# NethermindEth/starkpack-winterfell

Measured on AMD Instinct MI355X. Metric: trace-LDE + Merkle-commit field-ops/s (wall-clock ms in ms_per_step), 2^20x8 f64 trace blowup=8, higher is better.
Workload: dtype u64 (Goldilocks, Montgomery form) + u32 (BLAKE3)

## Files before the change

### starkpack-winterfell_amd/csrc/context.hip

```cpp
#include "wf_internal.hpp"

#include <atomic>

#include "field.hpp"

using namespace wf;

static thread_local char g_err[512] = "";

std::atomic<uint64_t> g_fail_epoch{0};
uint64_t fail_epoch() { return g_fail_epoch.load(std::memory_order_relaxed); }

int fail(int code, const char *fmt, ...) {
    g_fail_epoch.fetch_add(1, std::memory_order_relaxed);
    va_list ap;
    va_start(ap, fmt);
    vsnprintf(g_err, sizeof(g_err), fmt, ap);
    va_end(ap);
    return code;
}

const char *last_error_text() { return g_err; }

wf_tuning tuning_from_env() {
// ... 2 lines not shown
    if (!on || strcmp(on, "1") != 0) return t;
    if (const char *e = getenv("WF_EXP_MAX_DIGIT")) {
        const int v = atoi(e);
        if (v >= 4 && v <= 11) t.max_digit = (uint32_t)v;
    }
    t.no_specialized = getenv("WF_EXP_NO_SPECIALIZED") != nullptr;
    t.full_tiles = getenv("WF_EXP_FULL_TILES") != nullptr;
    t.no_fused_hash = getenv("WF_EXP_NO_FUSED_HASH") != nullptr;
    t.no_chunked = getenv("WF_EXP_NO_CHUNKED") != nullptr;
    t.persistent_always = getenv("WF_EXP_PERSISTENT_ALWAYS") != nullptr;
    t.no_persistent = getenv("WF_EXP_NO_PERSISTENT") != nullptr;
    if (const char *e = getenv("WF_EXP_MERKLE_L2_MIN")) {
        const int v = atoi(e);
        if (v >= 10 && v <= 30) t.merkle_l2_min = (uint32_t)v;
    }
    t.no_pipeline = getenv("WF_EXP_NO_PIPELINE") != nullptr;
    t.no_tail_pack = getenv("WF_EXP_NO_TAIL_PACK") != nullptr;
    t.no_coset_inner = getenv("WF_EXP_NO_COSET_INNER") != nullptr;
    t.no_gtab = getenv("WF_EXP_NO_GTAB") != nullptr;
    t.no_staged_chunks = getenv("WF_EXP_NO_STAGED_CHUNKS") != nullptr;
    t.no_gtab1 = getenv("WF_EXP_NO_GTAB1") != nullptr;
    t.no_ftab = getenv("WF_EXP_NO_FTAB") != nullptr;
    t.no_gtab1_wide = getenv("WF_EXP_NO_GTAB1_WIDE") != nullptr;
    t.gtab1_f64 = getenv("WF_EXP_GTAB1_F64") != nullptr;
    if (const char *e = getenv("WF_EXP_WIDE_TI")) {
        const int v = atoi(e);
        if (v == 1 || v == 2 || v == 4 || v == 8) t.wide_ti = (uint32_t)v;
    }
    if (const char *e = getenv("WF_EXP_PIPELINE_MIN_BYTES")) {
        const long long v = atoll(e);
        if (v >= 0 && v <= (1ll << 40)) t.pipeline_min_bytes = (size_t)v;
    }
    if (const char *e = getenv("WF_EXP_FAIL_AFTER_SEGMENT")) {
        const int v = atoi(e);
        if (v >= 0 && v < 4096) t.fail_after_segment = v;
    }
    if (const char *e = getenv("WF_EXP_GRIND_WINDOW_LOG2")) {
        const int v = atoi(e);
        if (v >= 2 && v <= 30) t.grind_window_log2 = (uint32_t)v;
    }
    if (const char *e = getenv("WF_EXP_GRIND_WINDOW_CAP_LOG2")) {
        const int v = atoi(e);
        if (v >= 2 && v <= 30) t.grind_window_cap_log2 = (uint32_t)v;
    }
    return t;
}
// ... 395 lines not shown
```

### starkpack-winterfell_amd/csrc/path.hip

```cpp
#include "wf_internal.hpp"

#include "kernels.hpp"
#include "keccak_dev.hpp"
#include "keccak_kernels.hpp"
#include "merkle_plan.hpp"
#include "rescue_kernels.hpp"
#include "rescue_jive_kernels.hpp"
#include "griffin_dev.hpp"
#include "seg_kernels.hpp"
#include "col_kernels.hpp"
#include "fri_kernels.hpp"
#include "tables.hpp"

using namespace wf;

#if defined(WF_EXPERIMENTS) && defined(WF_EXP_STAMPS)
static unsigned long long *g_exp_stamps = nullptr;
static unsigned long long *exp_stamps_buffer() {
    if (!g_exp_stamps && hipMalloc(&g_exp_stamps, 4096 * 8 * 8) == hipSuccess) (void)hipMemset(g_exp_stamps, 0, 4096 * 8 * 8);
    return g_exp_stamps;
}
extern "C" int wf_exp_stamps_read(unsigned long long *out, int clear) {
    if (!g_exp_stamps) return -1;
    if (hipMemcpy(out, g_exp_stamps, 4096 * 8 * 8, hipMemcpyDeviceToHost) != hipSuccess) return -2;
// ... 181 lines not shown
    return true;
}

template <class F>
struct SegDesc {
    typedef typename F::T T;
    const T *in;
    T *work;
    T *out;
    uint32_t logN, n_seg, n_cosets;
    bool rows_out;
    void *leaves = nullptr;
    uint32_t hash_epr = 0;
    uint32_t digest_words = 8;
    bool *fused = nullptr;
    const TableSet *pre;
    const T *fin_tab = nullptr;
    bool pad_traces = false;
    bool pad_in_kernel = false;
    uint32_t base_cols, total_base_cols, coset0;
    uint64_t row_width, trace_lde_elems;
    uint32_t seg0 = 0, seg_cnt = 0;
    int phase = 0;
};

template <class F>
static int run_seg_transform(wf_ctx *ctx, hipStream_t st, const SegDesc<F> &d) {
    typedef typename F::T T;
    const bool inverse = !d.rows_out;
    TableSet *tw;
    int rc = root_tables<F>(ctx, d.logN, inverse, &tw);
    if (rc) return rc;
    const Plan plan = seg_plan<F>(d.logN, d.n_seg, ctx->tune.max_digit, ctx->tune.full_tiles);
    const uint64_t N = (uint64_t)1 << d.logN;

    SegArgs<F> a;
    memset(&a, 0, sizeof(a));
    a.logN = d.logN;
    a.n_seg = d.n_seg;
    a.n_cosets = d.n_cosets;
    a.tw = as_pow2l<F>(*tw);
    if (d.pre) {
        a.pre = as_pow2l<F>(*d.pre);
        a.pre_lo_stride = d.pre->lo_stride;
        a.pre_hi_stride = d.pre->hi_stride;
    }
// ... 29 lines not shown
        const uint64_t tickets_tp = (uint64_t)(d.n_cosets / 2) << (d.logN - logDl);
        const uint64_t launch_rows = (uint64_t)d.n_cosets << d.logN;
        tailpack = logDl >= (ctx->tune.persistent_always || F::BYTES == 16 ? 7u : 9u) && logDl <= 10 && tickets_tp % 8 == 0 &&
                   tickets_tp < (1ull << 31) &&
                   (ctx->tune.persistent_always || launch_rows >= (1ull << 20));
    }
    T *work_tail = tailpack ? d.work + (size_t)d.n_cosets * nf * N * S_ : nullptr;

    const uint32_t run_cnt = tailpack ? nf : (d.seg_cnt ? d.seg_cnt : d.n_seg);
    const size_t run_off = (size_t)d.seg0 * (N * SegCfg<F>::S);
    a.seg_stride = tailpack ? nf : d.n_seg;
    uint32_t done_bits = 0;
    for (int pi = 0; pi + 1 < plan.n_pass; pi++) {
        if (d.phase == 2) {
            done_bits += plan.dig[pi];
            continue;
        }
        const bool first = pi == 0;
        a.logD = plan.dig[pi];
        a.O = (uint64_t)1 << done_bits;
        a.I = N >> (done_bits + a.logD);
        rc = digit_table<F>(ctx, a.logD, inverse, &a.digit_tw);
        if (rc) return rc;
        if (d.rows_out) {
            a.src = first ? d.in : d.work;
            a.dst = d.work;
            a.src_shared = first ? 1 : 0;
            a.pre_on = first ? 1 : 0;
            a.scale_on = 0;
        } else {
            a.src = first ? d.in : d.work;
            a.dst = d.work;
            a.src_shared = 0;
            a.pre_on = 0;
            a.scale_on = first ? 1 : 0;
            a.scale = inv_n;
        }
        a.src += run_off;
        a.dst += run_off;
        a.n_seg = run_cnt;
        uint32_t threads;
        size_t lds;
        rc = seg_launch_dims<F>(a.logD, threads, lds, false);
        if (rc) return rc;
        const uint64_t grid = (uint64_t)n_groups * run_cnt * a.O * a.I;
        if (grid > 0x7FFFFFFFull) return fail(WF_ERR_ARG, "problem too large for one launch (%llu groups)", (unsigned long long)grid);
// ... 90 lines not shown
    }
    a.n_seg = d.n_seg;
    a.seg_stride = d.n_seg;
    a.coset_inner = 0;
    a.fout_tab = nullptr;
    if (d.phase == 1) return 0;
    {
        const int pi = plan.n_pass - 1;
        const bool single = plan.n_pass == 1;
        a.logD = plan.dig[pi];
        a.O = (uint64_t)1 << done_bits;
        a.I = 1;
        a.n_prev = plan.n_pass - 1;
        for (int i = 0; i < pi; i++) a.prev_log[i] = plan.dig[i];
        rc = digit_table<F>(ctx, a.logD, inverse, &a.digit_tw);
        if (rc) return rc;
        a.src = single ? d.in : d.work;
        a.dst = d.out;
        a.src_shared = (single && d.rows_out) ? 1 : 0;
        a.pre_on = (single && d.rows_out) ? 1 : 0;
        a.fin_tab = (single && d.rows_out && !packed) ? d.fin_tab : nullptr;
        a.scale_on = (single && !d.rows_out) ? 1 : 0;
        a.scale = inv_n;
        uint32_t threads;
        size_t lds;
        rc = seg_launch_dims<F>(a.logD, threads, lds, true);
        if (rc) return rc;
        const uint64_t grid = (uint64_t)n_groups * d.n_seg * a.O;
        if (grid > 0x7FFFFFFFull) return fail(WF_ERR_ARG, "problem too large for one launch (%llu groups)", (unsigned long long)grid);
        const bool fuse_on = d.rows_out && d.leaves && !ctx->tune.no_fused_hash;
        const bool may_fuse = fuse_on && !packed;
        const bool chunked = d.n_seg > 16 && !ctx->tune.no_chunked;
        const uint32_t n_chunks = chunked ? (d.n_seg + 15) / 16 : 1;
        const uint64_t tickets = (uint64_t)d.n_cosets * a.O * n_chunks;
        const uint64_t launch_rows = (uint64_t)d.n_cosets << d.logN;
        const bool one_seg = d.n_seg == 1 && d.total_base_cols == d.base_cols;
        const bool always = ctx->tune.persistent_always;
        const bool persistent = may_fuse && !single && (d.n_seg <= 16 || chunked) && threads * 2 == (1u << a.logD) &&
                                (always || !one_seg || a.logD >= 10) &&
                                (always || one_seg || chunked || d.total_base_cols != d.base_cols || launch_rows >= (1ull << 20)) &&
                                tickets % 8 == 0 && tickets < (1ull << 31) && launch_rows * n_chunks * 32 < (1ull << 40) &&
                                !ctx->tune.no_persistent;
        const bool fuse_packed = fuse_on && packed && (F::BYTES == 16 || a.lg_log >= 2 || d.total_base_cols != d.base_cols);
        const bool fuse = persistent || (may_fuse && d.n_seg == 1 && d.total_base_cols == d.base_cols) || fuse_packed;
        a.leaves = fuse ? (uint32_t *)d.leaves : nullptr;
        a.hash_epr = d.hash_epr;
// ... 66 lines not shown
#endif
            void *kargs[] = {&a};
            HIP_TRY(hipLaunchKernel(kern, dim3((uint32_t)std::min<uint64_t>(tickets, resident)), dim3(threads), kargs, lds_p, st));
            if (chunked) {
                HIP_TRY(hipGetLastError());
                launch_merge_chunks(st, ctx->hash_tmp.p, n_chunks, launch_rows, d.leaves, a.digest_words);
            }
        } else if (d.rows_out && packed)
            hipLaunchKernelGGL((k_seg_last<F, SEG_OUT_ROWS, true>), dim3((uint32_t)grid), dim3(threads), lds, st, a);
        else {
            const void *kern = d.rows_out ? (const void *)k_seg_last<F, SEG_OUT_ROWS> : (const void *)k_seg_last<F, SEG_OUT_SEG>;
            constexpr bool F8 = F::BYTES == 8;
            if (F8 && threads * 2 == (1u << a.logD) && !ctx->tune.no_specialized) {
                if (a.logD == 10)
                    kern = d.rows_out ? (const void *)k_seg_last<F, SEG_OUT_ROWS, false, F8 ? 10 : 0> : (const void *)k_seg_last<F, SEG_OUT_SEG, false, F8 ? 10 : 0>;
                else if (a.logD == 9)
                    kern = d.rows_out ? (const void *)k_seg_last<F, SEG_OUT_ROWS, false, F8 ? 9 : 0> : (const void *)k_seg_last<F, SEG_OUT_SEG, false, F8 ? 9 : 0>;
            }
            if (lds > 64 * 1024) HIP_TRY(hipFuncSetAttribute(kern, hipFuncAttributeMaxDynamicSharedMemorySize, 160 * 1024));
            void *kargs[] = {&a};
            HIP_TRY(hipLaunchKernel(kern, dim3((uint32_t)grid), dim3(threads), kargs, lds, st));
        }
        HIP_TRY(hipGetLastError());
    }
    return 0;
}

template <class F>
static int run_xpose(wf_ctx *ctx, hipStream_t st, bool to_seg, const void *src, void *dst, uint64_t R, uint32_t W,
                     uint32_t total_base_cols, uint32_t n_seg, uint32_t seg0 = 0, uint32_t seg_cnt = 0) {
    if (seg_cnt == 0) seg_cnt = n_seg - seg0;
    XposeArgs<F> x;
    x.seg0 = seg0;
    x.src = (const typename F::T *)src;
    x.dst = (typename F::T *)dst;
    x.R = R;
    x.W = W;
    x.total_base_cols = total_base_cols;
    constexpr uint32_t RPB = XPOSE_TILES * 256 / SegCfg<F>::S;
    const uint64_t grid = (uint64_t)seg_cnt * ((R + RPB - 1) / RPB);
    if (grid > 0x7FFFFFFFull) return fail(WF_ERR_ARG, "problem too large for one launch");
    prof_mark(ctx, st, to_seg ? "layout.cols_to_segments" : "layout.segments_to_cols");
    if (to_seg)
        hipLaunchKernelGGL(k_cols_to_seg<F>, dim3((uint32_t)grid), dim3(256), 0, st, x);
    else
        hipLaunchKernelGGL(k_seg_to_cols<F>, dim3((uint32_t)grid), dim3(256), 0, st, x);
// ... 194 lines not shown
    d.seg0 = seg0;
    d.seg_cnt = seg_cnt;
    rc = run_seg_transform<F>(ctx, st, d);
    if (rc) return rc;
    if (phase == 1) return 0;

    if (d_leaves) {
        if (!hashed) {
            prof_mark(ctx, st, "hash_rows");
            rc = run_hash_rows<F>(ctx, st, d_lde, Nrows * row_width, Nrows, (uint32_t)row_width, base_cols, p->n_traces, d_leaves, p->hasher, p->digest_bytes);
            if (rc) return rc;
        }
        if (d_nodes) {
            prof_mark(ctx, st, "merkle");
            rc = run_merkle(ctx, st, d_leaves, Nrows, d_nodes, p->hasher, p->digest_bytes);
            if (rc) return rc;
        }
    }
    prof_mark(ctx, st, "between_calls");
    return 0;
}

template <class F>
static int trace_commit_dev(wf_ctx *ctx, const wf_params *p, const void *d_trace, void *d_polys, void *d_lde,
                            void *d_leaves, void *d_nodes, hipStream_t st, hipEvent_t input_read = nullptr) {
    PathBufs<F> b;
    int rc = path_buffers<F>(ctx, p, b);
    if (rc) return rc;
    const uint64_t R = (uint64_t)1 << p->log2_trace_len;
    rc = run_xpose<F>(ctx, st, true, d_trace, b.segA, R, p->ext_degree, b.total_base_cols, b.n_seg);
    if (rc) return rc;
    if (input_read) HIP_TRY(hipEventRecord(input_read, st));
    SegDesc<F> d;
    memset(&d, 0, sizeof(d));
    d.in = b.segA;
    d.work = b.segA;
    d.out = b.segB;
    d.logN = p->log2_trace_len;
    d.n_seg = b.n_seg;
    d.n_cosets = 1;
    d.rows_out = false;
    rc = run_seg_transform<F>(ctx, st, d);
    if (rc) return rc;
    rc = run_xpose<F>(ctx, st, false, b.segB, d_polys, R, p->ext_degree, b.total_base_cols, b.n_seg);
    if (rc) return rc;
    return evaluate_and_commit<F>(ctx, st, p, b, d_lde, d_leaves, d_nodes);
}

template <class F>
static int trace_commit_pipelined_impl(wf_ctx *ctx, const wf_params *p, const void *const *cols_in, void *d_stage, void *d_polys,
                                       void *d_lde, void *d_leaves, void *d_nodes, hipStream_t st, void *const *polys_out) {
    typedef typename F::T T;
    constexpr uint32_t S = SegCfg<F>::S;
    PathBufs<F> b;
    int rc = path_buffers<F>(ctx, p, b);
    if (rc) return rc;
    const uint64_t R = (uint64_t)1 << p->log2_trace_len;
    const size_t colb = R * sizeof(T), TC = b.total_base_cols;
    if (!ctx->copy_stream) HIP_TRY(hipStreamCreateWithFlags(&ctx->copy_stream, hipStreamNonBlocking));
    while (ctx->seg_events.size() < (size_t)b.n_seg + 1) {
        hipEvent_t e;
        HIP_TRY(hipEventCreateWithFlags(&e, hipEventDisableTiming));
        ctx->seg_events.push_back(e);
    }
    HIP_TRY(hipEventRecord(ctx->seg_events[b.n_seg], st));
// ... 107 lines not shown

int wf_constraint_commit_dev(wf_ctx *ctx, const wf_params *p, const void *d_polys, void *d_lde, void *d_leaves,
                             void *d_nodes, void *stream) {
    if (!ctx) return fail(WF_ERR_ARG, "ctx is null");
    int rc = check_params(p, true);
    if (rc) return rc;
    if (!d_polys || !d_lde) return fail(WF_ERR_ARG, "null device buffer");
    HIP_TRY(hipSetDevice(ctx->device));
    hipStream_t st = stream ? (hipStream_t)stream : ctx->stream;
    WF_ENTER(ctx, st);
    if (p->field == WF_FIELD_F64) return constraint_commit_dev<F64>(ctx, p, d_polys, d_lde, d_leaves, d_nodes, st);
    return constraint_commit_dev<F128>(ctx, p, d_polys, d_lde, d_leaves, d_nodes, st);
}

}

template <class F>
static int trace_commit_shard_dev(wf_ctx *ctx, const wf_params *p, uint32_t coset0, uint32_t n_cosets,
                                  const void *d_trace, void *d_polys, void *d_lde, void *d_leaves, hipStream_t st) {
    PathBufs<F> b;
    int rc = path_buffers<F>(ctx, p, b, n_cosets);
    if (rc) return rc;
    const uint64_t R = (uint64_t)1 << p->log2_trace_len;
    rc = run_xpose<F>(ctx, st, true, d_trace, b.segA, R, p->ext_degree, b.total_base_cols, b.n_seg);
    if (rc) return rc;
    SegDesc<F> d;
    memset(&d, 0, sizeof(d));
    d.in = b.segA;
    d.work = b.segA;
    d.out = b.segB;
    d.logN = p->log2_trace_len;
    d.n_seg = b.n_seg;
    d.n_cosets = 1;
    d.rows_out = false;
    rc = run_seg_transform<F>(ctx, st, d);
    if (rc) return rc;
    if (d_polys) {
        rc = run_xpose<F>(ctx, st, false, b.segB, d_polys, R, p->ext_degree, b.total_base_cols, b.n_seg);
        if (rc) return rc;
    }
    return evaluate_and_commit<F>(ctx, st, p, b, d_lde, d_leaves, nullptr, coset0, n_cosets);
}

extern "C" {

int wf_trace_commit_shard_dev(wf_ctx *ctx, const wf_params *p, uint32_t coset_begin, uint32_t coset_count,
                              const void *d_trace, void *d_polys, void *d_lde_shard, void *d_leaves_shard,
                              void *stream) {
    if (!ctx) return fail(WF_ERR_ARG, "ctx is null");
    int rc = check_params(p, false);
    if (rc) return rc;
    if ((rc = check_blake3_only(p, "wf_trace_commit_shard_dev"))) return rc;
    if (!d_trace || !d_lde_shard || !d_leaves_shard) return fail(WF_ERR_ARG, "null device buffer");
    const uint32_t blowup = 1u << p->log2_blowup;
    if (coset_count == 0 || coset_begin >= blowup || coset_count > blowup - coset_begin)
        return fail(WF_ERR_ARG, "coset range [%u, %u) is not inside [0, %u)", coset_begin, coset_begin + coset_count, blowup);
    HIP_TRY(hipSetDevice(ctx->device));
    hipStream_t st = stream ? (hipStream_t)stream : ctx->stream;
// ... 425 lines not shown
```

### starkpack-winterfell_amd/csrc/seg_kernels.hpp

```cpp
#pragma once

#include <hip/hip_runtime.h>
#include <stdint.h>

#include "field.hpp"
#include "kernels.hpp"

#ifndef WF_EXPERIMENTS
#undef WF_EXP_SKIP_LOAD
#undef WF_EXP_SKIP_NTT
#undef WF_EXP_SKIP_STORE
#undef WF_EXP_LOCAL_STORE
#undef WF_EXP_STAMPS
#endif

namespace wf {

template <class F>
struct SegCfg {
    static constexpr uint32_t S = 64 / F::BYTES;
    static constexpr uint32_t HP = S / 2;
    static constexpr bool RADIX16 = F::BYTES == 8;
    static constexpr bool RADIX8 = F::BYTES == 16;
    static constexpr uint32_t LOAD_BATCH = F::BYTES == 8 ? 8 : 4;
};

template <class T>
struct alignas(16) Pair {
// ... 11 lines not shown
    if (z & 1) {
        *pz++ = F::zero();
        z++;
    }
    const Pair<typename F::T> zz{F::zero(), F::zero()};
    for (; z < row_width; z += 2, pz += 2) store_pair(pz, zz);
}

template <class F>
__device__ __forceinline__ Pair<typename F::T> pair_from(const uint4 &qa, const uint4 &qb);
template <>
__device__ __forceinline__ Pair<uint64_t> pair_from<F64>(const uint4 &qa, const uint4 &) {
    Pair<uint64_t> v;
    v.a = ((uint64_t)qa.y << 32) | qa.x;
    v.b = ((uint64_t)qa.w << 32) | qa.z;
    return v;
}
template <>
__device__ __forceinline__ Pair<U128> pair_from<F128>(const uint4 &qa, const uint4 &qb) {
    Pair<U128> v;
    v.a = U128{((uint64_t)qa.y << 32) | qa.x, ((uint64_t)qa.w << 32) | qa.z};
    v.b = U128{((uint64_t)qb.y << 32) | qb.x, ((uint64_t)qb.w << 32) | qb.z};
    return v;
}

enum : int { SEG_OUT_SEG = 0, SEG_OUT_ROWS = 1 };

template <int LOGD>
__device__ __forceinline__ uint32_t tile_threads() {
    return LOGD ? (1u << (LOGD ? LOGD - 1 : 0)) : blockDim.x;
}
#define WF_TILE_BOUNDS(LOGD, GENERIC) __launch_bounds__((LOGD) ? (1 << ((LOGD) ? (LOGD) - 1 : 0)) : (GENERIC), (LOGD) ? 4 : 1)

__device__ __forceinline__ uint64_t xcd_group_index(uint64_t b, uint64_t total) {
    if ((total & 63) != 0) return b;
    const uint64_t xcd = b & 7, seq = b >> 3;
    return (((seq >> 3) << 3) + xcd) * 8 + (seq & 7);
}

__device__ __forceinline__ uint64_t coset_inner_split(uint64_t bid, uint32_t lc, uint32_t &c) {
    const uint64_t hi = bid >> 6;
    c = (uint32_t)hi & ((1u << lc) - 1);
    return ((hi >> lc) << 6) | (bid & 63);
}

__device__ __forceinline__ uint32_t ilog2_pow2(uint64_t v) { return 63u - (uint32_t)__builtin_clzll(v); }
// ... 20 lines not shown
    uint32_t scale_on;
    T scale;
    uint32_t n_prev;
    uint32_t prev_log[3];
    uint32_t base_cols;
    uint32_t total_base_cols;
    uint32_t store_cols, total_store_cols;
    uint32_t pad_traces;
    uint32_t tail_pad;
    uint32_t seg_stride;
    uint32_t coset0;
    uint32_t rows_per_k;
    uint32_t cpr_log, lg_log;
    uint64_t row_width;
    uint64_t trace_lde_elems;
    uint32_t *leaves;
    uint32_t hash_epr;
    uint32_t digest_words;
    uint32_t *chunk_cvs;
    uint32_t n_chunks;
    uint32_t *tile_counters;
    const T *src_tail;
    uint32_t tail_cols;
#ifdef WF_EXP_STAMPS
    unsigned long long *stamps;
#endif
};

#if defined(WF_EXPERIMENTS) && defined(WF_EXP_R8_NO_SPLIT)
constexpr uint32_t R8_SPLIT = 0;
#else
constexpr uint32_t R8_SPLIT = 4;
#endif
__host__ __device__ constexpr uint32_t radix8_rounds(uint32_t logD) {
    return (R8_SPLIT == 4 && logD >= 4 && logD % 3 == 1) ? logD / 3 - 1 : logD / 3;
}

template <class F>
__device__ __forceinline__ uint32_t seg_digit_reverse(uint32_t pos, uint32_t logD) {
    uint32_t k = 0, cur = logD, sh = 0;
    while (SegCfg<F>::RADIX16 && cur >= 4) {
        k |= ((pos >> (cur - 4)) & 15u) << sh;
        sh += 4;
        cur -= 4;
    }
    if (SegCfg<F>::RADIX8) {
// ... 656 lines not shown
    }
    const uint32_t pstride = NT >> hp_shift, pos0 = threadIdx.x >> hp_shift;
    if (pos0 >= D) return;
    const uint32_t k0 = seg_digit_reverse<F>(pos0, a.logD);
    T *dst_lane = dst + row0 * S + lane_a;
    const uint32_t k_shift = logI + (S == 8 ? 3 : 2);
    for (uint32_t pj = 0; pj < D; pj += pstride) {
        const uint32_t k = k0 | seg_digit_reverse<F>(pj, a.logD);
        P2 v = *reinterpret_cast<P2 *>(x + (pos0 + pj) * S + lane_a);
        const T f = aux[k];
        v.a = F::mul(v.a, f);
        v.b = F::mul(v.b, f);
        if (PACKED && a.pre_on) {
            v.a = F::mul(v.a, start_a);
            v.b = F::mul(v.b, start_b);
        }
#ifdef WF_EXP_SKIP_STORE
        if (*reinterpret_cast<const uint32_t *>(&v.a) == a.logN + 77777u)
#endif
        store_pair(dst_lane + ((uint64_t)k << k_shift), v);
    }
}

template <class F, int EVAL, int TI, int GTAB = 0, int LOGD = 0>
__global__ void __launch_bounds__(1024) k_seg_strided_wide(SegArgs<F> a) {
    if (LOGD) a.logD = LOGD;
    static_assert(SegCfg<F>::RADIX16 && TI >= 2 && (TI & (TI - 1)) == 0, "f64 tiles of 2, 4 or 8 inner positions");
    typedef typename F::T T;
    typedef Pair<T> P2;
    constexpr uint32_t S = SegCfg<F>::S, LANES = TI * S, HPW = LANES / 2;
    constexpr uint32_t LOGS = ilog2_const(S), LOGL = ilog2_const(LANES), LOGTI = ilog2_const(TI), LOGHPW = ilog2_const(HPW);
    extern __shared__ __attribute__((aligned(16))) unsigned char smem_raw[];
    const uint32_t D = 1u << a.logD, NT = blockDim.x;
    T *x = reinterpret_cast<T *>(smem_raw);
    T *twd = x + (size_t)D * LANES;
    T *fin = twd + D;
    T *fout = fin + D;

    uint64_t bid = xcd_group_index(blockIdx.x, gridDim.x);
    uint32_t c_in = 0;
    if (a.coset_inner) bid = coset_inner_split(bid, a.coset_inner - 1, c_in);
    const uint32_t logI = ilog2_pow2(a.I), logO = ilog2_pow2(a.O), logIt = logI - LOGTI;
    const uint64_t i0 = (bid & ((a.I >> LOGTI) - 1)) << LOGTI;
    const uint64_t o = (bid >> logIt) & (a.O - 1);
    const uint32_t rest = (uint32_t)(bid >> (logIt + logO));
    const uint32_t c = a.coset_inner ? c_in : rest / a.n_seg, g = a.coset_inner ? rest : rest - c * a.n_seg;
// ... 237 lines not shown
        tw_q[q] = a.digit_tw[kq[q]];
        if (!PACKED && a.fin_tab)
            fi_a[q] = fi_b[q] = a.fin_tab[((uint64_t)(a.coset0 + c) << a.logN) + kq[q]];
        else
            pin.fetch(kq[q], fi_a[q], fi_b[q]);
    }
    const uint4 twk0 = park(tw_q[0]), twk1 = park(tw_q[1]);
    uint4 r0, r1, r2, r3, r4, r5, r6, r7;
    r0 = r1 = r2 = r3 = r4 = r5 = r6 = r7 = make_uint4(0, 0, 0, 0);
#ifdef WF_EXP_SKIP_LOAD
#define WF_ITEM_PTR(WK) reinterpret_cast<const uint4 *>(a.src + 2 * (uint64_t)((WK) & 63))
#else
#define WF_ITEM_PTR(WK) reinterpret_cast<const uint4 *>(src + 2 * (uint64_t)(WK))
#endif
#define WF_LOAD_ITEM(U, RA, RB)                            \
    do {                                                   \
        const uint32_t wk_ = threadIdx.x + (U) * step;     \
        if (wk_ < nitems) {                                \
            const uint4 *p_ = WF_ITEM_PTR(wk_);            \
            RA = p_[0];                                    \
            if (F::BYTES == 16) RB = p_[1];                \
        }                                                  \
    } while (0)
    if (from_regs) {
        if (F::BYTES == 8) {
            WF_LOAD_ITEM(0, r0, r0);
            WF_LOAD_ITEM(1, r1, r1);
            WF_LOAD_ITEM(2, r2, r2);
            WF_LOAD_ITEM(3, r3, r3);
            WF_LOAD_ITEM(4, r4, r4);
            WF_LOAD_ITEM(5, r5, r5);
            WF_LOAD_ITEM(6, r6, r6);
            WF_LOAD_ITEM(7, r7, r7);
        } else {
            WF_LOAD_ITEM(0, r0, r1);
            WF_LOAD_ITEM(1, r2, r3);
            WF_LOAD_ITEM(2, r4, r5);
            WF_LOAD_ITEM(3, r6, r7);
        }
    }
#undef WF_LOAD_ITEM
#undef WF_ITEM_PTR
#pragma unroll
    for (uint32_t q = 0; q < 2; q++) {
        if (threadIdx.x + q * NT < D) {
            if (scale_in)
                aux[kq[q]] = (!PACKED && a.fin_tab) ? fi_a[q] : F::mul(fi_a[q], fi_b[q]);
            else
                twd[kq[q]] = unpark<F>(q == 0 ? twk0 : twk1);
        }
    }
    __syncthreads();
    if (PACKED && a.pre_on) {
        for (uint32_t wk = threadIdx.x; wk < nitems; wk += NT) {
            P2 v;
            const uint32_t d = wk >> hp_shift;
            const uint32_t lgm = (1u << a.lg_log) - 1, cola = lane_a & lgm, colb = lane_b & lgm;
            const T *srow = src + (uint64_t)d * S;
            const T fa = pre_a.get(d);
            const T fb = a.lg_log ? fa : pre_b.get(d);
            v.a = act_a ? F::mul(srow[cola], fa) : F::zero();
            v.b = act_b ? F::mul(srow[colb], fb) : F::zero();
            *reinterpret_cast<P2 *>(x + 2 * wk) = v;
        }
    } else {
#define WF_FILL_ITEM(U, RA, RB)                                \
    do {                                                       \
        const uint32_t wk_ = threadIdx.x + (U) * step;         \
        if (wk_ < nitems) {                                    \
            P2 v_ = pair_from<F>(RA, RB);                      \
            if (a.pre_on) {                                    \
                const T f_ = aux[wk_ >> hp_shift];             \
                v_.a = F::mul(v_.a, f_);                       \
                v_.b = F::mul(v_.b, f_);                       \
            }                                                  \
            *reinterpret_cast<P2 *>(x + 2 * wk_) = v_;         \
        }                                                      \
    } while (0)
        if (F::BYTES == 8) {
            WF_FILL_ITEM(0, r0, r0);
            WF_FILL_ITEM(1, r1, r1);
            WF_FILL_ITEM(2, r2, r2);
            WF_FILL_ITEM(3, r3, r3);
            WF_FILL_ITEM(4, r4, r4);
            WF_FILL_ITEM(5, r5, r5);
            WF_FILL_ITEM(6, r6, r6);
            WF_FILL_ITEM(7, r7, r7);
// ... 751 lines not shown
```

### starkpack-winterfell_amd/csrc/tables.hpp

```cpp
#pragma once

#include "wf_internal.hpp"

#include "pow2l.hpp"

using namespace wf;

static int table_upload(wf_ctx *ctx, void **dst, const void *src, size_t bytes) {
    *dst = nullptr;
    hipError_t e = dev_malloc(ctx, dst, bytes);
    if (e != hipSuccess) return fail(WF_ERR_HIP, "table allocation of %zu bytes failed: %s", bytes, hipGetErrorString(e));
    e = hipMemcpy(*dst, src, bytes, hipMemcpyHostToDevice);
    if (e != hipSuccess) {
        (void)hipFree(*dst);
        *dst = nullptr;
        return fail(WF_ERR_HIP, "table upload failed: %s", hipGetErrorString(e));
    }
    return 0;
}

template <class F>
static int upload_pow2l(wf_ctx *ctx, const std::vector<typename F::T> &bases, uint32_t logN, TableSet &ts) {
    typedef typename F::T T;
    const uint32_t s = (logN + 1) / 2;
// ... 174 lines not shown
        if (inverse) w = f_inv<F>(w);
        const uint64_t D = (uint64_t)1 << logD, I = (uint64_t)1 << logI;
        const T base = f_pow<F>(w, (u128)1 << (logN - logD - logI));
        std::vector<T> tab(D * I);
        T step = F::one();
        for (uint64_t i = 0; i < I; i++) {
            T acc = F::one();
            for (uint64_t k = 0; k < D; k++) {
                tab[i * D + k] = acc;
                acc = F::mul(acc, step);
            }
            step = F::mul(step, base);
        }
        TableSet ts;
        const int rcu = table_upload(ctx, &ts.lo, tab.data(), tab.size() * sizeof(T));
        if (rcu) return rcu;
        it = ctx->tables.emplace(key, ts).first;
    }
    *out = (const typename F::T *)it->second.lo;
    return 0;
}

template <class F>
static typename F::T offset_elem(const wf_params *p, uint64_t &lo, uint64_t &hi) {
    u128 off;
    memcpy(&off, p->domain_offset, 16);
    lo = (uint64_t)off;
    hi = (uint64_t)(off >> 64);
    return F::from_u128_canonical(off);
}
```

### starkpack-winterfell_amd/csrc/wf_internal.hpp

```cpp
#pragma once

#include "../../include/wf_lde.h"

#include <hip/hip_runtime.h>

#include <algorithm>
#include <atomic>
#include <cstdarg>
#include <cstdio>
#include <cstring>
#include <map>
#include <mutex>
#include <set>
#include <string>
#include <thread>
#include <tuple>
#include <type_traits>
#include <vector>

int fail(int code, const char *fmt, ...) __attribute__((format(printf, 2, 3)));
const char *last_error_text();
uint64_t fail_epoch();

#define HIP_TRY(expr)                                                                              \
// ... 11 lines not shown
    void *lo = nullptr, *hi = nullptr;
    uint32_t s = 0, mask = 0;
    uint64_t lo_stride = 0, hi_stride = 0;
};

struct wf_tuning {
    uint32_t max_digit = 0;
    bool full_tiles = false;
    bool no_specialized = false;
    bool no_fused_hash = false;
    bool no_chunked = false;
    bool persistent_always = false;
    bool no_persistent = false;
    uint32_t merkle_l2_min = 18;
    bool no_pipeline = false;
    size_t pipeline_min_bytes = (size_t)1 << 20;
    bool no_tail_pack = false;
    bool no_coset_inner = false;
    bool no_gtab1_wide = false;
    bool no_ftab = false;
    bool no_gtab1 = false;
    bool gtab1_f64 = false;
    bool no_staged_chunks = false;
    bool no_gtab = false;
    uint32_t wide_ti = 0;
    int fail_after_segment = -1;
    uint32_t grind_window_log2 = 0;
    uint32_t grind_window_cap_log2 = 0;
};
wf_tuning tuning_from_env();

struct wf_ctx {
    int device = 0;
    int num_cus = 256;
    wf_tuning tune;
    uint32_t digest_bytes = 32;
    uint32_t hasher = WF_HASH_BLAKE3;
    DevBuf pack_tmp;
    hipStream_t stream = nullptr;
    std::map<std::tuple<int, int, int, int, uint64_t, uint64_t>, TableSet> tables;
    int prof_level = 0;
    bool prof_on = false;
    std::vector<hipEvent_t> prof_ev;
    std::vector<const char *> prof_name;
    size_t prof_n = 0;
    DevBuf scratch;
// ... 182 lines not shown
```

Baseline: 2082 billion.

## Interpolate trace columns directly from column layout, skipping input transpose

Adds a column-tiled inverse NTT route that reads the trace directly in its original column-major layout. A new first-pass kernel applies the inverse-n scaling and twiddle factors from a precomputed factor table, and the final pass gathers from a column-index mapping. This removes the separate transpose of the input into segment layout before interpolation. In exchange the new kernel does strided global reads and adds a new table, and it only applies to base-field plans with one or two passes.

```diff
diff --git a/starkpack-winterfell_amd/csrc/context.hip b/starkpack-winterfell_amd/csrc/context.hip
--- a/starkpack-winterfell_amd/csrc/context.hip
+++ b/starkpack-winterfell_amd/csrc/context.hip
@@ -48,6 +48,7 @@
     t.no_gtab1 = getenv("WF_EXP_NO_GTAB1") != nullptr;
     t.no_ftab = getenv("WF_EXP_NO_FTAB") != nullptr;
     t.no_gtab1_wide = getenv("WF_EXP_NO_GTAB1_WIDE") != nullptr;
+    t.no_col_interp = getenv("WF_EXP_NO_COL_INTERP") != nullptr;
     t.gtab1_f64 = getenv("WF_EXP_GTAB1_F64") != nullptr;
     if (const char *e = getenv("WF_EXP_WIDE_TI")) {
         const int v = atoi(e);
diff --git a/starkpack-winterfell_amd/csrc/interp_cols_map.hpp b/starkpack-winterfell_amd/csrc/interp_cols_map.hpp
--- /dev/null
+++ b/starkpack-winterfell_amd/csrc/interp_cols_map.hpp
@@ -0,0 +1,22 @@
+#pragma once
+#include <stdint.h>
+
+#if defined(__HIPCC__) || defined(__CUDACC__)
+#define WF_MAP_HD __host__ __device__
+#else
+#define WF_MAP_HD
+#endif
+
+namespace wf {
+
+WF_MAP_HD inline uint64_t interp_cols_index(uint32_t logN, uint32_t logI, uint32_t logS, uint32_t g, uint64_t t, uint32_t l,
+                                            uint64_t i) {
+    return ((((((uint64_t)g << (logN - logI)) + t) << logS) + l) << logI) + i;
+}
+
+inline bool interp_cols_route_ok(uint32_t ext_degree, int n_pass, uint32_t logN, uint32_t last_digit, uint32_t logS) {
+    if (ext_degree != 1 || n_pass < 1 || n_pass > 2 || logN < 1) return false;
+    return n_pass == 1 ? last_digit == logN : (last_digit >= logS && last_digit < logN);
+}
+
+}
diff --git a/starkpack-winterfell_amd/csrc/path.hip b/starkpack-winterfell_amd/csrc/path.hip
--- a/starkpack-winterfell_amd/csrc/path.hip
+++ b/starkpack-winterfell_amd/csrc/path.hip
@@ -227,6 +227,8 @@
     uint64_t row_width, trace_lde_elems;
     uint32_t seg0 = 0, seg_cnt = 0;
     int phase = 0;
+    const T *cols = nullptr;
+    hipEvent_t cols_read = nullptr;
 };
 
 template <class F>
@@ -302,6 +304,32 @@
         a.I = N >> (done_bits + a.logD);
         rc = digit_table<F>(ctx, a.logD, inverse, &a.digit_tw);
         if (rc) return rc;
+        if (d.cols) {
+            constexpr uint32_t LOGS = ilog2_const(SegCfg<F>::S);
+            const uint32_t logI = d.logN - done_bits - a.logD;
+            a.src = d.cols;
+            a.dst = d.work;
+            rc = interp_cols_factor_table<F>(ctx, d.logN, a.logD, logI, LOGS, &a.fcol_tab);
+            if (rc) return rc;
+            const uint32_t threads = (uint32_t)std::min<size_t>(1024, std::max<size_t>(64, ((size_t)1 << a.logD) / 2));
+            const size_t lds = (((size_t)SegCfg<F>::S + 1) << a.logD) * sizeof(T);
+            const uint64_t grid = (uint64_t)d.total_base_cols * a.O * (a.I >> LOGS);
+            if (grid > 0x7FFFFFFFull) return fail(WF_ERR_ARG, "problem too large for one launch (%llu groups)", (unsigned long long)grid);
+            const void *kern = (const void *)k_seg_strided_cols<F>;
+            constexpr bool F8 = F::BYTES == 8;
+            if (F8 && threads * 2 == (1u << a.logD) && !ctx->tune.no_specialized) {
+                if (a.logD == 10) kern = (const void *)k_seg_strided_cols<F, F8 ? 10 : 0>;
+                if (a.logD == 9) kern = (const void *)k_seg_strided_cols<F, F8 ? 9 : 0>;
+            }
+            if (lds > 64 * 1024) HIP_TRY(hipFuncSetAttribute(kern, hipFuncAttributeMaxDynamicSharedMemorySize, 160 * 1024));
+            prof_mark(ctx, st, tag_s);
+            void *kargs[] = {&a};
+            HIP_TRY(hipLaunchKernel(kern, dim3((uint32_t)grid), dim3(threads), kargs, lds, st));
+            HIP_TRY(hipGetLastError());
+            if (d.cols_read) HIP_TRY(hipEventRecord(d.cols_read, st));
+            done_bits += a.logD;
+            continue;
+        }
         if (d.rows_out) {
             a.src = first ? d.in : d.work;
             a.dst = d.work;
@@ -438,6 +466,10 @@
         a.fin_tab = (single && d.rows_out && !packed) ? d.fin_tab : nullptr;
         a.scale_on = (single && !d.rows_out) ? 1 : 0;
         a.scale = inv_n;
+        if (d.cols) {
+            a.col_fill = 1;
+            if (single) a.src = d.cols;
+        }
         uint32_t threads;
         size_t lds;
         rc = seg_launch_dims<F>(a.logD, threads, lds, true);
@@ -550,6 +582,7 @@
             HIP_TRY(hipLaunchKernel(kern, dim3((uint32_t)grid), dim3(threads), kargs, lds, st));
         }
         HIP_TRY(hipGetLastError());
+        if (d.cols && single && d.cols_read) HIP_TRY(hipEventRecord(d.cols_read, st));
     }
     return 0;
 }
@@ -790,15 +823,18 @@
 }
 
 template <class F>
-static int trace_commit_dev(wf_ctx *ctx, const wf_params *p, const void *d_trace, void *d_polys, void *d_lde,
-                            void *d_leaves, void *d_nodes, hipStream_t st, hipEvent_t input_read = nullptr) {
-    PathBufs<F> b;
-    int rc = path_buffers<F>(ctx, p, b);
-    if (rc) return rc;
+static int interpolate_columns(wf_ctx *ctx, hipStream_t st, const wf_params *p, const PathBufs<F> &b, const void *d_trace,
+                               hipEvent_t input_read = nullptr) {
+    typedef typename F::T T;
     const uint64_t R = (uint64_t)1 << p->log2_trace_len;
-    rc = run_xpose<F>(ctx, st, true, d_trace, b.segA, R, p->ext_degree, b.total_base_cols, b.n_seg);
-    if (rc) return rc;
-    if (input_read) HIP_TRY(hipEventRecord(input_read, st));
+    const Plan plan = seg_plan<F>(p->log2_trace_len, b.n_seg, ctx->tune.max_digit, ctx->tune.full_tiles);
+    const bool col_tiles = !ctx->tune.no_col_interp &&
+                           interp_cols_route_ok(p->ext_degree, plan.n_pass, p->log2_trace_len, plan.dig[plan.n_pass - 1], ilog2_const(SegCfg<F>::S));
+    if (!col_tiles) {
+        int rc = run_xpose<F>(ctx, st, true, d_trace, b.segA, R, p->ext_degree, b.total_base_cols, b.n_seg);
+        if (rc) return rc;
+        if (input_read) HIP_TRY(hipEventRecord(input_read, st));
+    }
     SegDesc<F> d;
     memset(&d, 0, sizeof(d));
     d.in = b.segA;
@@ -808,7 +844,22 @@
     d.n_seg = b.n_seg;
     d.n_cosets = 1;
     d.rows_out = false;
-    rc = run_seg_transform<F>(ctx, st, d);
+    if (col_tiles) {
+        d.cols = (const T *)d_trace;
+        d.cols_read = input_read;
+        d.total_base_cols = b.total_base_cols;
+    }
+    return run_seg_transform<F>(ctx, st, d);
+}
+
+template <class F>
+static int trace_commit_dev(wf_ctx *ctx, const wf_params *p, const void *d_trace, void *d_polys, void *d_lde,
+                            void *d_leaves, void *d_nodes, hipStream_t st, hipEvent_t input_read = nullptr) {
+    PathBufs<F> b;
+    int rc = path_buffers<F>(ctx, p, b);
+    if (rc) return rc;
+    const uint64_t R = (uint64_t)1 << p->log2_trace_len;
+    rc = interpolate_columns<F>(ctx, st, p, b, d_trace, input_read);
     if (rc) return rc;
     rc = run_xpose<F>(ctx, st, false, b.segB, d_polys, R, p->ext_degree, b.total_base_cols, b.n_seg);
     if (rc) return rc;
@@ -962,18 +1013,7 @@
     int rc = path_buffers<F>(ctx, p, b, n_cosets);
     if (rc) return rc;
     const uint64_t R = (uint64_t)1 << p->log2_trace_len;
-    rc = run_xpose<F>(ctx, st, true, d_trace, b.segA, R, p->ext_degree, b.total_base_cols, b.n_seg);
-    if (rc) return rc;
-    SegDesc<F> d;
-    memset(&d, 0, sizeof(d));
-    d.in = b.segA;
-    d.work = b.segA;
-    d.out = b.segB;
-    d.logN = p->log2_trace_len;
-    d.n_seg = b.n_seg;
-    d.n_cosets = 1;
-    d.rows_out = false;
-    rc = run_seg_transform<F>(ctx, st, d);
+    rc = interpolate_columns<F>(ctx, st, p, b, d_trace);
     if (rc) return rc;
     if (d_polys) {
         rc = run_xpose<F>(ctx, st, false, b.segB, d_polys, R, p->ext_degree, b.total_base_cols, b.n_seg);
diff --git a/starkpack-winterfell_amd/csrc/seg_kernels.hpp b/starkpack-winterfell_amd/csrc/seg_kernels.hpp
--- a/starkpack-winterfell_amd/csrc/seg_kernels.hpp
+++ b/starkpack-winterfell_amd/csrc/seg_kernels.hpp
@@ -4,6 +4,7 @@
 #include <stdint.h>
 
 #include "field.hpp"
+#include "interp_cols_map.hpp"
 #include "kernels.hpp"
 
 #ifndef WF_EXPERIMENTS
@@ -61,6 +62,22 @@
     v.a = U128{((uint64_t)qa.y << 32) | qa.x, ((uint64_t)qa.w << 32) | qa.z};
     v.b = U128{((uint64_t)qb.y << 32) | qb.x, ((uint64_t)qb.w << 32) | qb.z};
     return v;
+}
+
+template <class F>
+__device__ __forceinline__ void store_col_item(typename F::T *pa, typename F::T *pb, bool swap, const uint4 &qa, const uint4 &qb);
+template <>
+__device__ __forceinline__ void store_col_item<F64>(uint64_t *pa, uint64_t *pb, bool swap, const uint4 &qa, const uint4 &) {
+    const uint2 first = make_uint2(swap ? qa.z : qa.x, swap ? qa.w : qa.y), second = make_uint2(swap ? qa.x : qa.z, swap ? qa.y : qa.w);
+    *reinterpret_cast<uint2 *>(swap ? pb : pa) = first;
+    *reinterpret_cast<uint2 *>(swap ? pa : pb) = second;
+}
+template <>
+__device__ __forceinline__ void store_col_item<F128>(U128 *pa, U128 *pb, bool swap, const uint4 &qa, const uint4 &qb) {
+    const uint4 first = make_uint4(swap ? qb.x : qa.x, swap ? qb.y : qa.y, swap ? qb.z : qa.z, swap ? qb.w : qa.w);
+    const uint4 second = make_uint4(swap ? qa.x : qb.x, swap ? qa.y : qb.y, swap ? qa.z : qb.z, swap ? qa.w : qb.w);
+    *reinterpret_cast<uint4 *>(swap ? pb : pa) = first;
+    *reinterpret_cast<uint4 *>(swap ? pa : pb) = second;
 }
 
 enum : int { SEG_OUT_SEG = 0, SEG_OUT_ROWS = 1 };
@@ -127,6 +144,8 @@
     uint32_t *tile_counters;
     const T *src_tail;
     uint32_t tail_cols;
+    uint32_t col_fill;
+    const T *fcol_tab;
 #ifdef WF_EXP_STAMPS
     unsigned long long *stamps;
 #endif
@@ -829,6 +848,141 @@
     }
 }
 
+template <class F, int LOGD = 0>
+__global__ void WF_TILE_BOUNDS(LOGD, 1024) k_seg_strided_cols(SegArgs<F> a) {
+    typedef typename F::T T;
+    if (LOGD) a.logD = LOGD;
+    const uint32_t NT = tile_threads<LOGD>();
+    typedef Pair<T> P2;
+    constexpr uint32_t S = SegCfg<F>::S, HP = SegCfg<F>::HP, LOGS = ilog2_const(S);
+    constexpr uint32_t hp_shift = HP == 4 ? 2 : 1;
+    extern __shared__ __attribute__((aligned(16))) unsigned char smem_raw[];
+    const uint32_t D = 1u << a.logD;
+    T *x = reinterpret_cast<T *>(smem_raw);
+    T *twd = x + (size_t)D * S;
+
+    const uint64_t bid = xcd_group_index(blockIdx.x, gridDim.x);
+    const uint32_t logI = ilog2_pow2(a.I), logO = ilog2_pow2(a.O), logIt = logI - LOGS;
+    const uint64_t ib = bid & ((a.I >> LOGS) - 1), i0 = ib << LOGS;
+    const uint64_t o = (bid >> logIt) & (a.O - 1);
+    const uint32_t B = (uint32_t)(bid >> (logIt + logO));
+    const T *src = a.src + ((uint64_t)B << a.logN) + ((o << a.logD) << logI) + i0;
+
+    const uint32_t nitems = D * HP, step = NT;
+    uint32_t kq[2];
+    T tw_q[2];
+#pragma unroll
+    for (uint32_t q = 0; q < 2; q++) {
+        const uint32_t k = threadIdx.x + q * NT;
+        kq[q] = k < D ? k : D - 1;
+        tw_q[q] = a.digit_tw[kq[q]];
+    }
+    const bool direct = SegCfg<F>::RADIX16 && a.logD >= 4;
+    const uint32_t m16 = D >> 4, l16 = threadIdx.x & (S - 1), j16 = threadIdx.x / S;
+    const bool has16 = threadIdx.x < m16 * S;
+    T vr[16];
+    uint4 r0, r1, r2, r3, r4, r5, r6, r7;
+    r0 = r1 = r2 = r3 = r4 = r5 = r6 = r7 = make_uint4(0, 0, 0, 0);
+    if (direct) {
+        if (has16) {
+            const T *pr = src + ((uint64_t)j16 << logI) + l16;
+            const uint64_t rstep = (uint64_t)m16 << logI;
+#pragma unroll
+            for (uint32_t q = 0; q < 16; q++) {
+                vr[q] = *pr;
+                pr += rstep;
+            }
+        }
+    } else {
+#define WF_LOAD_ITEM(U, RA, RB)                                                                                              \
+    do {                                                                                                                     \
+        const uint32_t wk_ = threadIdx.x + (U) * step;                                                                       \
+        if (wk_ < nitems) {                                                                                                  \
+            const uint4 *p_ = reinterpret_cast<const uint4 *>(src + ((uint64_t)(wk_ >> hp_shift) << logI) + 2 * (wk_ & (HP - 1))); \
+            RA = p_[0];                                                                                                      \
+            if (F::BYTES == 16) RB = p_[1];                                                                                  \
+        }                                                                                                                    \
+    } while (0)
+        if (F::BYTES == 8) {
+            WF_LOAD_ITEM(0, r0, r0);
+            WF_LOAD_ITEM(1, r1, r1);
+            WF_LOAD_ITEM(2, r2, r2);
+            WF_LOAD_ITEM(3, r3, r3);
+            WF_LOAD_ITEM(4, r4, r4);
+            WF_LOAD_ITEM(5, r5, r5);
+            WF_LOAD_ITEM(6, r6, r6);
+            WF_LOAD_ITEM(7, r7, r7);
+        } else {
+            WF_LOAD_ITEM(0, r0, r1);
+            WF_LOAD_ITEM(1, r2, r3);
+            WF_LOAD_ITEM(2, r4, r5);
+            WF_LOAD_ITEM(3, r6, r7);
+        }
+#undef WF_LOAD_ITEM
+    }
+#pragma unroll
+    for (uint32_t q = 0; q < 2; q++)
+        if (threadIdx.x + q * NT < D) twd[kq[q]] = tw_q[q];
+    if (!direct) {
+#define WF_FILL_ITEM(U, RA, RB)                                                            \
+    do {                                                                                   \
+        const uint32_t wk_ = threadIdx.x + (U) * step;                                     \
+        if (wk_ < nitems) *reinterpret_cast<P2 *>(x + 2 * wk_) = pair_from<F>(RA, RB);     \
+    } while (0)
+        if (F::BYTES == 8) {
+            WF_FILL_ITEM(0, r0, r0);
+            WF_FILL_ITEM(1, r1, r1);
+            WF_FILL_ITEM(2, r2, r2);
+            WF_FILL_ITEM(3, r3, r3);
+            WF_FILL_ITEM(4, r4, r4);
+            WF_FILL_ITEM(5, r5, r5);
+            WF_FILL_ITEM(6, r6, r6);
+            WF_FILL_ITEM(7, r7, r7);
+        } else {
+            WF_FILL_ITEM(0, r0, r1);
+            WF_FILL_ITEM(1, r2, r3);
+            WF_FILL_ITEM(2, r4, r5);
+            WF_FILL_ITEM(3, r6, r7);
+        }
+#undef WF_FILL_ITEM
+    }
+    __syncthreads();
+    const uint32_t pstride = NT >> hp_shift, pos0 = threadIdx.x >> hp_shift, lane_a = 2 * (threadIdx.x & (HP - 1));
+    const uint32_t k0 = seg_digit_reverse<F>(pos0 < D ? pos0 : 0, a.logD);
+    const T *fc = a.fcol_tab + ((ib << a.logD) << LOGS) + lane_a;
+    seg_lds_ntt<F, -1, (LOGD ? (1u << LOGD) : 0u)>(x, twd, a.logD, NT, vr, direct);
+
+    if (pos0 >= D) return;
+    T *dst = a.dst + interp_cols_index(a.logN, logI, LOGS, B >> LOGS, o << a.logD, B & (S - 1), i0 + lane_a);
+    const uint32_t k_shift = LOGS + logI;
+    if constexpr (LOGD != 0 && F::BYTES == 8) {
+        uint32_t kk[8];
+        uint4 ff[8];
+#pragma unroll
+        for (uint32_t j = 0; j < 8; j++) {
+            kk[j] = k0 | seg_digit_reverse<F>(j * pstride, a.logD);
+            ff[j] = *reinterpret_cast<const uint4 *>(fc + ((uint64_t)kk[j] << LOGS));
+        }
+#pragma unroll
+        for (uint32_t j = 0; j < 8; j++) {
+            P2 v = *reinterpret_cast<P2 *>(x + (pos0 + j * pstride) * S + lane_a);
+            const P2 f = pair_from<F>(ff[j], ff[j]);
+            v.a = F::mul(v.a, f.a);
+            v.b = F::mul(v.b, f.b);
+            store_pair(dst + ((uint64_t)kk[j] << k_shift), v);
+        }
+        return;
+    }
+    for (uint32_t pj = 0; pj < D; pj += pstride) {
+        const uint32_t k = k0 | seg_digit_reverse<F>(pj, a.logD);
+        P2 v = *reinterpret_cast<P2 *>(x + (pos0 + pj) * S + lane_a);
+        const P2 f = *reinterpret_cast<const P2 *>(fc + ((uint64_t)k << LOGS));
+        v.a = F::mul(v.a, f.a);
+        v.b = F::mul(v.b, f.b);
+        store_pair(dst + ((uint64_t)k << k_shift), v);
+    }
+}
+
 template <class F, int EVAL, int TI, int GTAB = 0, int LOGD = 0>
 __global__ void __launch_bounds__(1024) k_seg_strided_wide(SegArgs<F> a) {
     if (LOGD) a.logD = LOGD;
@@ -1112,7 +1266,36 @@
             if (F::BYTES == 16) RB = p_[1];                \
         }                                                  \
     } while (0)
-    if (from_regs) {
+    constexpr uint32_t LOGS = ilog2_const(S);
+    const bool col_fill = OUT == SEG_OUT_SEG && !PACKED && a.col_fill != 0;
+#define WF_LOAD_COL_ITEM(U, RA, RB)                                                                                         \
+    do {                                                                                                                    \
+        const uint32_t wk_ = threadIdx.x + (U) * step, l_ = wk_ & (S - 1);                                                  \
+        if (wk_ < nitems && g * S + l_ < a.total_base_cols) {                                                               \
+            const uint4 *p_ = reinterpret_cast<const uint4 *>(                                                              \
+                a.src + interp_cols_index(a.logN, logD_, LOGS, g, o, l_, 2 * (uint64_t)(wk_ >> LOGS)));                     \
+            RA = p_[0];                                                                                                     \
+            if (F::BYTES == 16) RB = p_[1];                                                                                 \
+        }                                                                                                                   \
+    } while (0)
+    if (col_fill) {
+        if (F::BYTES == 8) {
+            WF_LOAD_COL_ITEM(0, r0, r0);
+            WF_LOAD_COL_ITEM(1, r1, r1);
+            WF_LOAD_COL_ITEM(2, r2, r2);
+            WF_LOAD_COL_ITEM(3, r3, r3);
+            WF_LOAD_COL_ITEM(4, r4, r4);
+            WF_LOAD_COL_ITEM(5, r5, r5);
+            WF_LOAD_COL_ITEM(6, r6, r6);
+            WF_LOAD_COL_ITEM(7, r7, r7);
+        } else {
+            WF_LOAD_COL_ITEM(0, r0, r1);
+            WF_LOAD_COL_ITEM(1, r2, r3);
+            WF_LOAD_COL_ITEM(2, r4, r5);
+            WF_LOAD_COL_ITEM(3, r6, r7);
+        }
+#undef WF_LOAD_COL_ITEM
+    } else if (from_regs) {
         if (F::BYTES == 8) {
             WF_LOAD_ITEM(0, r0, r0);
             WF_LOAD_ITEM(1, r1, r1);
@@ -1153,6 +1336,32 @@
             v.b = act_b ? F::mul(srow[colb], fb) : F::zero();
             *reinterpret_cast<P2 *>(x + 2 * wk) = v;
         }
+    } else if (col_fill) {
+#define WF_FILL_COL_ITEM(U, RA, RB)                                                   \
+    do {                                                                              \
+        const uint32_t wk_ = threadIdx.x + (U) * step;                                \
+        if (wk_ < nitems) {                                                           \
+            const uint32_t l_ = wk_ & (S - 1), p_ = wk_ >> LOGS;                      \
+            const uint32_t ea_ = 2 * p_ * S + l_;                                     \
+            store_col_item<F>(x + ea_, x + ea_ + S, (p_ & 1u) != 0, RA, RB);          \
+        }                                                                             \
+    } while (0)
+        if (F::BYTES == 8) {
+            WF_FILL_COL_ITEM(0, r0, r0);
+            WF_FILL_COL_ITEM(1, r1, r1);
+            WF_FILL_COL_ITEM(2, r2, r2);
+            WF_FILL_COL_ITEM(3, r3, r3);
+            WF_FILL_COL_ITEM(4, r4, r4);
+            WF_FILL_COL_ITEM(5, r5, r5);
+            WF_FILL_COL_ITEM(6, r6, r6);
+            WF_FILL_COL_ITEM(7, r7, r7);
+        } else {
+            WF_FILL_COL_ITEM(0, r0, r1);
+            WF_FILL_COL_ITEM(1, r2, r3);
+            WF_FILL_COL_ITEM(2, r4, r5);
+            WF_FILL_COL_ITEM(3, r6, r7);
+        }
+#undef WF_FILL_COL_ITEM
     } else {
 #define WF_FILL_ITEM(U, RA, RB)                                \
     do {                                                       \
diff --git a/starkpack-winterfell_amd/csrc/tables.hpp b/starkpack-winterfell_amd/csrc/tables.hpp
--- a/starkpack-winterfell_amd/csrc/tables.hpp
+++ b/starkpack-winterfell_amd/csrc/tables.hpp
@@ -220,6 +220,35 @@
 }
 
 template <class F>
+static int interp_cols_factor_table(wf_ctx *ctx, uint32_t logN, uint32_t logD, uint32_t logI, uint32_t logS, const typename F::T **out) {
+    auto key = std::make_tuple((int)F::FIELD_ID, (int)logN, 9, (int)(logD | (logI << 8) | (logS << 16)), (uint64_t)0, (uint64_t)0);
+    auto it = ctx->tables.find(key);
+    if (it == ctx->tables.end()) {
+        typedef typename F::T T;
+        const T w = f_inv<F>(f_root_of_unity<F>(logN ? logN : 1));
+        const T inv_n = f_inv<F>(F::from_u128_canonical((u128)1 << logN));
+        const uint64_t D = (uint64_t)1 << logD, I = (uint64_t)1 << logI, S = (uint64_t)1 << logS;
+        const T base = f_pow<F>(w, (u128)1 << (logN - logD - logI));
+        std::vector<T> tab(D * I);
+        T step = F::one();
+        for (uint64_t i = 0; i < I; i++) {
+            T acc = inv_n;
+            for (uint64_t k = 0; k < D; k++) {
+                tab[(((i >> logS) << logD) + k) * S + (i & (S - 1))] = acc;
+                acc = F::mul(acc, step);
+            }
+            step = F::mul(step, base);
+        }
+        TableSet ts;
+        const int rcu = table_upload(ctx, &ts.lo, tab.data(), tab.size() * sizeof(T));
+        if (rcu) return rcu;
+        it = ctx->tables.emplace(key, ts).first;
+    }
+    *out = (const typename F::T *)it->second.lo;
+    return 0;
+}
+
+template <class F>
 static typename F::T offset_elem(const wf_params *p, uint64_t &lo, uint64_t &hi) {
     u128 off;
     memcpy(&off, p->domain_offset, 16);
diff --git a/starkpack-winterfell_amd/csrc/wf_internal.hpp b/starkpack-winterfell_amd/csrc/wf_internal.hpp
--- a/starkpack-winterfell_amd/csrc/wf_internal.hpp
+++ b/starkpack-winterfell_amd/csrc/wf_internal.hpp
@@ -57,6 +57,7 @@
     bool no_gtab1 = false;
     bool gtab1_f64 = false;
     bool no_staged_chunks = false;
+    bool no_col_interp = false;
     bool no_gtab = false;
     uint32_t wide_ti = 0;
     int fail_after_segment = -1;
```

Result: slower. 2005 billion (-3.7%).
